# PRBonn/SHINE_mapping

Measured on NVIDIA H100. Metric: sdf_train_points_per_sec_fwd_bwd, higher is better.
Workload: dtype f32

## Files before the change

shine_mapping_b200/csrc/shine_b200.cu:

```cuda

#include <cuda_runtime.h>
#include <math.h>
#include <stdint.h>

#include "shine_b200.h"

#ifndef SHINE_GATHER_GROUP
#define SHINE_GATHER_GROUP 2
#endif
#ifndef SHINE_TRAIN_MINB
#define SHINE_TRAIN_MINB 2
#endif
#ifndef SHINE_TRAIN_DECGRAD_MINB
#define SHINE_TRAIN_DECGRAD_MINB 1
#endif
#ifndef SHINE_INFER_MINB
#define SHINE_INFER_MINB 3
#endif

#include "shine_device.cuh"

namespace {


// ... 222 lines not shown
    const float s0 = odd ? v[0] : v[2], s1 = odd ? v[1] : v[3];
    const float r0 = __shfl_xor_sync(kFull, s0, 1), r1 = __shfl_xor_sync(kFull, s1, 1);
    if (!odd) { a[0] = v[0]; a[2] = v[1]; a[1] = r0; a[3] = r1; }
    else      { a[0] = r0;   a[2] = r1;   a[1] = v[2]; a[3] = v[3]; }
}
__device__ __forceinline__ void from_cfrag(const float (&c)[4], int odd, float (&v)[4]) {
    const float s0 = odd ? c[0] : c[2], s1 = odd ? c[1] : c[3];
    const float r0 = __shfl_xor_sync(kFull, s0, 1), r1 = __shfl_xor_sync(kFull, s1, 1);
    if (!odd) { v[0] = c[0]; v[1] = c[1]; v[2] = r0; v[3] = r1; }
    else      { v[0] = r0;   v[1] = r1;   v[2] = c[2]; v[3] = c[3]; }
}

#define SHINE_ACC_DECL float dW2[2][4][4], dW1[2][4], db2p[4][2], db1p[4][2], dw3p[4][2]

__device__ __forceinline__ float reduce_scatter_g8(const float (&v)[8], int lane) {
    float a[4], b[2];
    const bool b4 = (lane & 16) != 0, b3 = (lane & 8) != 0, b2 = (lane & 4) != 0;
#pragma unroll
    for (int i = 0; i < 4; ++i) a[i] = (b4 ? v[4 + i] : v[i]) + __shfl_xor_sync(kFull, b4 ? v[i] : v[4 + i], 16);
#pragma unroll
    for (int i = 0; i < 2; ++i) b[i] = (b3 ? a[2 + i] : a[i]) + __shfl_xor_sync(kFull, b3 ? a[i] : a[2 + i], 8);
    return (b2 ? b[1] : b[0]) + __shfl_xor_sync(kFull, b2 ? b[0] : b[1], 4);
}

__device__ __forceinline__ int frag_chunk(int lane) { return lane ^ ((lane >> 2) & 6); }
template <int NTF>
__device__ __forceinline__ void load_afrag(const float* blk, int c, AFrag<NTF>& a) {
    const float4 v = *reinterpret_cast<const float4*>(blk + 4 * c);
    a.set_packed(v.x, v.y, v.z, v.w);
}
__device__ __forceinline__ void load_bfrag(const float* blk, int c, uint2& bh, uint2& bl) {
    const float2 v = *reinterpret_cast<const float2*>(blk + 2 * c);
    split_fast2(v.x, v.y, bh.x, bh.y, bl.x, bl.y);
}
__device__ __forceinline__ void stage_afrags(float* blk, const int (&sq)[2], const float (&c)[4][4]) {
#pragma unroll
    for (int mt = 0; mt < 2; ++mt)
#pragma unroll
        for (int q = 0; q < 2; ++q)
            *reinterpret_cast<float4*>(blk + 128 * mt + 4 * sq[q]) = make_float4(c[2 * mt][q], c[2 * mt + 1][q], c[2 * mt][2 + q], c[2 * mt + 1][2 + q]);
}
__device__ __forceinline__ int xfrag_word(int ks, int c) { return 64 * ks + 2 * (c ^ (8 * ks)); }
__device__ __forceinline__ void load_xfrag(const float* sx, int ks, int c, uint2& bh, uint2& bl) {
    const float2 v = *reinterpret_cast<const float2*>(sx + xfrag_word(ks, c));
    split_fast2(v.x, v.y, bh.x, bh.y, bl.x, bl.y);
}


constexpr int kGatherGroup = SHINE_GATHER_GROUP;

using shine_internal::StepParams;

struct SmemPlan {
    static constexpr int W1 = 0;
    static constexpr int W1T = W1 + 2 * kH * kF;
    static constexpr int W2 = W1T + 2 * kF * kWS;
    static constexpr int W3W2T = W2 + 2 * kH * kWS;
    static constexpr int B1 = W3W2T + 2 * kH * kWS;
    static constexpr int B2 = B1 + kH;
    static constexpr int W3 = B2 + kH;
    static constexpr int B3 = W3 + kH;
    static constexpr int GSCALE = B3 + 1;
    static constexpr int kDecGradFloats = kH * kF + kH + kH * kH + kH + kH + 1;
    static constexpr int ZSUM = B3 + 4;
    static constexpr int kZsumFloats = 8 * 5 * kTile;
    static constexpr int STAGE = ZSUM + kZsumFloats;
    static constexpr int SB2 = 0;
    static constexpr int SU = SB2;
    static constexpr int SA1 = SB2 + kTile * kH;
    static constexpr int SX = SA1 + kTile * kH;
    static constexpr int SA2 = SX + kTile * kF;
    static constexpr int SDP = SA2;
    static constexpr int kStagePerWarp = SA2 + kTile * kH;
    static constexpr int kStageGrouped = SDP + 2 * kTile;
    __host__ __device__ static constexpr int stage_per_warp(bool grouped) { return grouped ? kStageGrouped : kStagePerWarp; }
    static constexpr int kGroupPerLevel = 4 * kTile;
    static constexpr int kW2Part = kH * kH;
};

constexpr int kMaxGroupedRuns = 6;

__device__ __forceinline__ void red_add_f2(float* p, float a, float b) {
    asm volatile("red.global.add.v2.f32 [%0], {%1,%2};" ::"l"(p), "f"(a), "f"(b) : "memory");
}
__device__ __forceinline__ int group_slot(int p) { return 4 * (p & 3) + (p >> 2); }

template <int LMAX>
__device__ __forceinline__ void grouped_scatter(const StepParams& P, int L, int tile, const float* __restrict__ pt,
                                                float* __restrict__ dtile, const float (&dxc)[4], int lane) {
    const int g = lane >> 2, t = lane & 3;
    *reinterpret_cast<float2*>(dtile + g * kF + 2 * t) = make_float2(dxc[0], dxc[1]);
    *reinterpret_cast<float2*>(dtile + (g + 8) * kF + 2 * t) = make_float2(dxc[2], dxc[3]);
    __syncwarp();
    uint2 bh[2], bl[2];
#pragma unroll
    for (int c = 0; c < 2; ++c)
        split_fast2(dtile[(8 * c + t) * kF + g], dtile[(8 * c + t + 4) * kF + g], bh[c].x, bh[c].y, bl[c].x, bl[c].y);
    const float sx = (g & 4) ? 1.f : -1.f, ox = (g & 4) ? 0.f : 1.f;
    const float sy = (g & 2) ? 1.f : -1.f, oy = (g & 2) ? 0.f : 1.f;
    const float sz = (g & 1) ? 1.f : -1.f, oz = (g & 1) ? 0.f : 1.f;
    const int id_off = 8 * (g & 1) + 4 + (g >> 1);
    const int own = group_slot(lane & 15);
#pragma unroll
    for (int i = 0; i < LMAX; ++i) {
        if (i >= L) break;
        const float* lt = pt + i * SmemPlan::kGroupPerLevel;
        const int v_own = __float_as_int(lt[48 + own]);
        const uint32_t same = __match_any_sync(kFull, v_own);
        const int lead = __ffs(same) - 1;
        const uint32_t bmask = __ballot_sync(kFull, v_own >= 0 && lead == lane);
        if (bmask == 0) continue;
        const int rid_own = v_own >= 0 ? __popc(bmask & ((1u << lead) - 1u)) : 255;
        const shine_level& lv = P.oct.lv[i];
        const int32_t* slot_words = reinterpret_cast<const int32_t*>(lv.hash_slots);
        float* gb = grad_base(lv, (uint32_t)tile, kF);
        const int nruns = __popc(bmask);
        if (nruns > kMaxGroupedRuns) {
            const int odd = t & 1, half = t >> 1, mp = group_slot(g + 8 * odd);
// ... 28 lines not shown
        {
            const f2_t s_x = f2_pack(sx, sx), o_x = f2_pack(ox, ox), s_y = f2_pack(sy, sy), o_y = f2_pack(oy, oy);
            const f2_t s_z = f2_pack(sz, sz), o_z = f2_pack(oz, oz);
            const f2_t X01 = f2_fma(f2_pack(tx4.x, tx4.y), s_x, o_x), X23 = f2_fma(f2_pack(tx4.z, tx4.w), s_x, o_x);
            const f2_t Y01 = f2_fma(f2_pack(ty4.x, ty4.y), s_y, o_y), Y23 = f2_fma(f2_pack(ty4.z, ty4.w), s_y, o_y);
            const f2_t Z01 = f2_fma(f2_pack(tz4.x, tz4.y), s_z, o_z), Z23 = f2_fma(f2_pack(tz4.z, tz4.w), s_z, o_z);
            f2_unpack(f2_mul(f2_mul(X01, Y01), Z01), w[0], w[1]);
            f2_unpack(f2_mul(f2_mul(X23, Y23), Z23), w[2], w[3]);
        }
        int rid[4];
#pragma unroll
        for (int q = 0; q < 4; ++q) rid[q] = __shfl_sync(kFull, rid_own, t + 4 * q);
        uint32_t rem = bmask;
        for (int r = 0; r < nruns; r += 2) {
            const int p1 = __ffs(rem) - 1; rem &= rem - 1;
            const int p2 = rem ? __ffs(rem) - 1 : p1; rem &= rem - 1;
            const int v1 = __shfl_sync(kFull, v_own, p1);
            const int v2 = (r + 1 < nruns) ? __shfl_sync(kFull, v_own, p2) : -1;
            AFrag<3> a0, a1;
            a0.set(rid[0] == r ? w[0] : 0.f, rid[0] == r + 1 ? w[0] : 0.f, rid[1] == r ? w[1] : 0.f, rid[1] == r + 1 ? w[1] : 0.f);
            a1.set(rid[2] == r ? w[2] : 0.f, rid[2] == r + 1 ? w[2] : 0.f, rid[3] == r ? w[3] : 0.f, rid[3] == r + 1 ? w[3] : 0.f);
            float c0[4] = {0.f, 0.f, 0.f, 0.f}, c1[4] = {0.f, 0.f, 0.f, 0.f};
            mma3x2<3>(c0, c1, a0, a1, bh[0], bl[0], bh[1], bl[1]);
            if (v1 >= 0) {
                const int row = __ldg(slot_words + 16 * (int64_t)v1 + id_off);
                red_add_f2(gb + (int64_t)row * kF + 2 * t, c0[0] + c1[0], c0[1] + c1[1]);
            }
            if (v2 >= 0) {
                const int row = __ldg(slot_words + 16 * (int64_t)v2 + id_off);
                red_add_f2(gb + (int64_t)row * kF + 2 * t, c0[2] + c1[2], c0[3] + c1[3]);
            }
        }
    }
    __syncwarp();
}

template <int NTF, bool TRAIN, bool DEC_GRAD, int LMAX, bool GROUPED = false>
__global__ void __launch_bounds__(256, !TRAIN ? SHINE_INFER_MINB : (DEC_GRAD && !GROUPED) ? SHINE_TRAIN_DECGRAD_MINB : SHINE_TRAIN_MINB)
sdf_fused_kernel(const __grid_constant__ StepParams P) {
    static_assert(!GROUPED || TRAIN, "the grouped scatter belongs to the training kernels");
    static_assert(!DEC_GRAD || TRAIN, "decoder gradients belong to the training kernels");
    static_assert(SmemPlan::kStagePerWarp >= SmemPlan::kDecGradFloats, "a warp's staging area holds its partial decoder gradient");
    static_assert(SmemPlan::kStageGrouped >= kH * kF + 3 * kH + 1, "a grouped warp's staging area holds its partial bias / dW1 gradients");
    static_assert(!(GROUPED && DEC_GRAD) ||
                      (SmemPlan::STAGE + 8 * (SmemPlan::kStageGrouped + LMAX * SmemPlan::kGroupPerLevel + SmemPlan::kW2Part)) * 4 + 1024 <=
                          227 * 1024 / SHINE_TRAIN_MINB,
                  "the grouped kernel's shared memory fits SHINE_TRAIN_MINB blocks/SM");
    extern __shared__ __align__(16) float smem[];
    uint32_t* smu = reinterpret_cast<uint32_t*>(smem);
    const int tid = threadIdx.x, lane = tid & 31, warp = tid >> 5;
    const int g = lane >> 2, t = lane & 3, odd = t & 1, half = t >> 1;
    constexpr int kWarps = 8;

    for (int i = tid; i < kH * kF; i += blockDim.x) {
        const int nrow = i / kF, k = i % kF;
        uint32_t hi, lo; split_tf32(P.dec.w1[i], hi, lo);
        smu[SmemPlan::W1 + i] = hi; smu[SmemPlan::W1 + kH * kF + i] = lo;
        smu[SmemPlan::W1T + k * kWS + nrow] = hi; smu[SmemPlan::W1T + kF * kWS + k * kWS + nrow] = lo;
    }
    for (int i = tid; i < kH * kH; i += blockDim.x) {
        const int nrow = i / kH, k = i % kH;
        const float w = P.dec.w2[i];
        uint32_t hi, lo; split_tf32(w, hi, lo);
        smu[SmemPlan::W2 + nrow * kWS + k] = hi; smu[SmemPlan::W2 + kH * kWS + nrow * kWS + k] = lo;
        split_tf32(__fmul_rn(P.dec.w3[nrow], w), hi, lo);
        smu[SmemPlan::W3W2T + k * kWS + nrow] = hi; smu[SmemPlan::W3W2T + kH * kWS + k * kWS + nrow] = lo;
    }
    if (tid < kH) {
        smem[SmemPlan::B1 + tid] = P.dec.b1 ? P.dec.b1[tid] : 0.f;
        smem[SmemPlan::B2 + tid] = P.dec.b2 ? P.dec.b2[tid] : 0.f;
        smem[SmemPlan::W3 + tid] = P.dec.w3[tid];
    }
    if (tid == 0) {
        smem[SmemPlan::B3] = P.dec.b3 ? P.dec.b3[0] : 0.f;
        smem[SmemPlan::GSCALE] = P.loss_scale * ((TRAIN && P.d_loss) ? __ldg(P.d_loss) : 1.0f);
    }
    constexpr int kPark = LMAX <= 4 ? 16 : 32;
    constexpr int kIdPark = 4 * LMAX;
    __syncthreads();
    SHINE_ACC_DECL;
#pragma unroll
    for (int a = 0; a < 2; ++a) {
#pragma unroll
        for (int b = 0; b < 4; ++b) { dW2[a][b][0] = dW2[a][b][1] = dW2[a][b][2] = dW2[a][b][3] = 0.f; }
        dW1[a][0] = dW1[a][1] = dW1[a][2] = dW1[a][3] = 0.f;
    }
#pragma unroll
    for (int j = 0; j < 4; ++j) { db2p[j][0] = db2p[j][1] = db1p[j][0] = db1p[j][1] = dw3p[j][0] = dw3p[j][1] = 0.f; }
    float dw3acc = 0.f, db2acc[4] = {0.f, 0.f, 0.f, 0.f}, db1acc[2][2] = {{0.f, 0.f}, {0.f, 0.f}};

    constexpr bool kSectorProbe = !TRAIN;
    const bool poly = P.oct.poly_interp != 0;
    const int L = P.oct.num_levels;

    float db3p = 0.f;
    float loss_acc = 0.f;

    constexpr int kStage = SmemPlan::stage_per_warp(GROUPED);
    float* stage = smem + SmemPlan::STAGE + warp * kStage;
    float* stX = stage + SmemPlan::SX;
    const int kp = g >> 2, fc = frag_chunk(lane);
    const int sq[2] = {frag_chunk(8 * t + (g & 3)), frag_chunk(8 * t + 4 + (g & 3))};
    float* gpt = smem + SmemPlan::STAGE + (DEC_GRAD ? 8 * kStage : 0) +
                 warp * (LMAX * SmemPlan::kGroupPerLevel + (DEC_GRAD ? 0 : kTile * kF));
    float* gdx = DEC_GRAD ? stX : gpt + LMAX * SmemPlan::kGroupPerLevel;
    float* w2p = smem + SmemPlan::STAGE + 8 * kStage + 8 * LMAX * SmemPlan::kGroupPerLevel + warp * SmemPlan::kW2Part;
    if (DEC_GRAD && GROUPED) {
#pragma unroll
        for (int f = 0; f < 8; ++f) *reinterpret_cast<float4*>(w2p + 128 * f + 4 * lane) = make_float4(0.f, 0.f, 0.f, 0.f);
    }

    const int warp_global = blockIdx.x * kWarps + warp;
    const int warp_stride = gridDim.x * kWarps;

    bool consecutive = true;
#pragma unroll
    for (int i = 1; i < LMAX; ++i)
        if (i < L && P.oct.lv[i].level != P.oct.lv[0].level - i) consecutive = false;

// ... 165 lines not shown
            for (int i = 0; i < kIdPark; ++i) idp[i] = __int_as_float(-1);
#pragma unroll
            for (int i = 0; i < LMAX; ++i) {
                if (GROUPED && i < L && half) gpt[i * SmemPlan::kGroupPerLevel + 48 + group_slot(g + 8 * odd)] = __int_as_float(slot[i]);
                if (i < L && slot[i] >= 0) {
                    const shine_level& lv = P.oct.lv[i];
                    const HashSlot* slots = reinterpret_cast<const HashSlot*>(lv.hash_slots);
                    hitmask |= 1u << i;
                    const int4 id4 = ldg_i4(slot_ids(slots, slot[i], half));
                    idp[4 * i] = __int_as_float(id4.x); idp[4 * i + 1] = __int_as_float(id4.y);
                    idp[4 * i + 2] = __int_as_float(id4.z); idp[4 * i + 3] = __int_as_float(id4.w);
                    float r0[8], r1[8], r2[8], r3[8];
                    ldg_row8(lv.features + (int64_t)id4.x * kF, r0);
                    ldg_row8(lv.features + (int64_t)id4.y * kF, r1);
                    ldg_row8(lv.features + (int64_t)id4.z * kF, r2);
                    ldg_row8(lv.features + (int64_t)id4.w * kF, r3);
                    Blend b; b.init(x, y, z, lv.level, poly);
                    pk[3 * i] = b.tx; pk[3 * i + 1] = b.ty; pk[3 * i + 2] = b.tz;
                    if (GROUPED) {
                        float* lt = gpt + i * SmemPlan::kGroupPerLevel + group_slot(g + 8 * odd);
                        if (half) lt[32] = b.tz; else { lt[0] = b.tx; lt[16] = b.ty; }
                    }
                    const float wz = half ? b.tz : b.uz;
                    const float w0 = __fmul_rn(__fmul_rn(b.ux, b.uy), wz), w1 = __fmul_rn(__fmul_rn(b.ux, b.ty), wz);
                    const float w2 = __fmul_rn(__fmul_rn(b.tx, b.uy), wz), w3 = __fmul_rn(__fmul_rn(b.tx, b.ty), wz);
                    blend4(acc, r0, r1, r2, r3, w0, w1, w2, w3);
                }
            }
#pragma unroll
            for (int q = 0; q < 4; ++q) {
                const float send = half ? acc[q] : acc[4 + q];
                const float recv = __shfl_xor_sync(kFull, send, 2);
                feat[q] = (half ? acc[4 + q] : acc[q]) + recv;
            }
        }
        }
        if (phase == 1 && __ballot_sync(kFull, hitmask != 0u) == 0u) {
            if (!TRAIN && P.mask && half == 0 && valid) P.mask[myp] = 0;
            if (P.pred && half == 0 && valid) P.pred[myp] = pred0;
            if (P.label != nullptr && valid) {
                float li, dpz;
                bce_point(pred0, lab, wgt, li, dpz);
                if (half == 0) { loss_acc += wgt * li; zsum += dpz; }
            }
            continue;
        }
        if (!TRAIN && P.mask) {
            bool present = false;
#pragma unroll
            for (int i = 0; i < LMAX; ++i) present = (i == P.mask_level) ? (((hitmask >> i) & 1u) != 0) : present;
            if (half == 0 && valid) P.mask[myp] = (uint8_t)present;
        }

        AFrag<NTF> ax;
        {
            float a[4]; to_afrag(feat, odd, a);
            ax.set(a[0], a[1], a[2], a[3]);
        }
        if (DEC_GRAD) {
#pragma unroll
            for (int q = 0; q < 4; ++q) stX[xfrag_word(kp, frag_chunk(16 * half + 4 * q + (g & 3))) + odd] = feat[q];
        }
        float h1[4][4];
        uint32_t m1 = 0;
        {
            uint2 bh[4], bl[4];
#pragma unroll
            for (int j = 0; j < 4; ++j) {
                const float bA = smem[SmemPlan::B1 + 8 * j + 2 * t], bB = smem[SmemPlan::B1 + 8 * j + 2 * t + 1];
                h1[j][0] = bA; h1[j][1] = bB; h1[j][2] = bA; h1[j][3] = bB;
                const int off = (8 * j + g) * kF + 2 * t;
                bh[j] = *reinterpret_cast<const uint2*>(smu + SmemPlan::W1 + off);
                bl[j] = *reinterpret_cast<const uint2*>(smu + SmemPlan::W1 + kH * kF + off);
            }
            mma3x4<NTF>(h1, ax, bh, bl);
#pragma unroll
            for (int j = 0; j < 4; ++j) {
#pragma unroll
                for (int r = 0; r < 4; ++r) {
                    if (TRAIN && h1[j][r] > 0.f) m1 |= 1u << (4 * j + r);
                    h1[j][r] = fmaxf(h1[j][r], 0.f);
                }
                if (DEC_GRAD && !GROUPED) {
#pragma unroll
                    for (int q = 0; q < 2; ++q)
                        *reinterpret_cast<float2*>(stage + SmemPlan::SB2 + (4 * kp + j) * 64 + 2 * sq[q]) = make_float2(h1[j][q], h1[j][2 + q]);
                }
            }
            if (DEC_GRAD && GROUPED) stage_afrags(stage + SmemPlan::SU + 256 * kp, sq, h1);
        }
        float h2[4][4];
        {
#pragma unroll
            for (int j = 0; j < 4; ++j) {
                const float bA = smem[SmemPlan::B2 + 8 * j + 2 * t], bB = smem[SmemPlan::B2 + 8 * j + 2 * t + 1];
                h2[j][0] = bA; h2[j][1] = bB; h2[j][2] = bA; h2[j][3] = bB;
            }
#pragma unroll
            for (int kk = 0; kk < 4; ++kk) {
                AFrag<NTF> a; a.set(h1[kk][0], h1[kk][2], h1[kk][1], h1[kk][3]);
                uint2 bh[4], bl[4];
#pragma unroll
                for (int j = 0; j < 4; ++j) {
                    const int off = (8 * j + g) * kWS + 8 * kk + 2 * t;
                    bh[j] = *reinterpret_cast<const uint2*>(smu + SmemPlan::W2 + off);
                    bl[j] = *reinterpret_cast<const uint2*>(smu + SmemPlan::W2 + kH * kWS + off);
                }
                mma3x4<NTF>(h2, a, bh, bl);
            }
#pragma unroll
            for (int j = 0; j < 4; ++j) {
#pragma unroll
                for (int r = 0; r < 4; ++r) h2[j][r] = fmaxf(h2[j][r], 0.f);
            }
        }
        float w3a[4], w3b[4];
#pragma unroll
        for (int j = 0; j < 4; ++j) { w3a[j] = smem[SmemPlan::W3 + 8 * j + 2 * t]; w3b[j] = smem[SmemPlan::W3 + 8 * j + 2 * t + 1]; }
        float p0 = 0.f, p8 = 0.f;
#pragma unroll
        for (int j = 0; j < 4; ++j) {
            p0 = fmaf(h2[j][0], w3a[j], p0); p0 = fmaf(h2[j][1], w3b[j], p0);
            p8 = fmaf(h2[j][2], w3a[j], p8); p8 = fmaf(h2[j][3], w3b[j], p8);
        }
        p0 += __shfl_xor_sync(kFull, p0, 1); p0 += __shfl_xor_sync(kFull, p0, 2);
        p8 += __shfl_xor_sync(kFull, p8, 1); p8 += __shfl_xor_sync(kFull, p8, 2);
        const float b3 = smem[SmemPlan::B3];
        p0 += b3; p8 += b3;
        const float pown = odd ? p8 : p0;
        if (phase == 0) { pred0 = pown; phase = 1; continue; }
        if (P.pred && half == 0 && valid) P.pred[myp] = pown;

        if (P.label == nullptr) continue;

        float dpo = 0.f;
        if (valid) {
            float li;
            bce_point(pown, lab, wgt, li, dpo);
            if (half == 0) loss_acc += wgt * li;
        }
        if (!TRAIN) continue;
        if (phase == 2) dpo = (g == 0 && odd == 0) ? zsum : 0.f;

        const float dpx = __shfl_xor_sync(kFull, dpo, 1);
        const float dp0 = odd ? dpx : dpo, dp8 = odd ? dpo : dpx;
        float db1t[4][2], dw3t[4][2];
        if (DEC_GRAD) {
#pragma unroll
            for (int j = 0; j < 4; ++j) { dw3t[j][0] = dp0 * h2[j][0] + dp8 * h2[j][2];  dw3t[j][1] = dp0 * h2[j][1] + dp8 * h2[j][3]; }
        }
        if (DEC_GRAD && !GROUPED) {
            float dh2[4][4];
#pragma unroll
            for (int j = 0; j < 4; ++j) {
                dh2[j][0] = h2[j][0] > 0.f ? dp0 * w3a[j] : 0.f; dh2[j][1] = h2[j][1] > 0.f ? dp0 * w3b[j] : 0.f;
                dh2[j][2] = h2[j][2] > 0.f ? dp8 * w3a[j] : 0.f; dh2[j][3] = h2[j][3] > 0.f ? dp8 * w3b[j] : 0.f;
                db2p[j][0] += dh2[j][0] + dh2[j][2]; db2p[j][1] += dh2[j][1] + dh2[j][3];
            }
            stage_afrags(stage + SmemPlan::SA2 + 256 * kp, sq, dh2);
        }
        if (DEC_GRAD && GROUPED) {
            uint32_t mg = 0, mg8 = 0;
#pragma unroll
            for (int j = 0; j < 4; ++j)
#pragma unroll
                for (int q = 0; q < 2; ++q) {
                    mg |= (h2[j][q] > 0.f ? 1u : 0u) << (8 * j + 2 * t + q);
                    mg8 |= (h2[j][2 + q] > 0.f ? 1u : 0u) << (8 * j + 2 * t + q);
                }
            mg |= __shfl_xor_sync(kFull, mg, 1); mg8 |= __shfl_xor_sync(kFull, mg8, 1);
            mg |= __shfl_xor_sync(kFull, mg, 2); mg8 |= __shfl_xor_sync(kFull, mg8, 2);
            if (t == 0) {
                *reinterpret_cast<float2*>(stage + SmemPlan::SDP + 2 * g) = make_float2(dp0, __uint_as_float(mg));
                *reinterpret_cast<float2*>(stage + SmemPlan::SDP + 2 * (g + 8)) = make_float2(dp8, __uint_as_float(mg8));
            }
        }
        if (DEC_GRAD && t == 0) db3p += dp0 + dp8;

        float dh1[4][4];
        {
#pragma unroll
            for (int j = 0; j < 4; ++j) { dh1[j][0] = dh1[j][1] = dh1[j][2] = dh1[j][3] = 0.f; }
#pragma unroll
            for (int kk = 0; kk < 4; ++kk) {
                const uint32_t a[4] = {h2[kk][0] > 0.f ? kTf32One : 0u, h2[kk][2] > 0.f ? kTf32One : 0u,
                                       h2[kk][1] > 0.f ? kTf32One : 0u, h2[kk][3] > 0.f ? kTf32One : 0u};
                uint2 bh[4], bl[4];
#pragma unroll
                for (int j = 0; j < 4; ++j) {
                    const int off = (8 * j + g) * kWS + 8 * kk + 2 * t;
                    bh[j] = *reinterpret_cast<const uint2*>(smu + SmemPlan::W3W2T + off);
                    bl[j] = *reinterpret_cast<const uint2*>(smu + SmemPlan::W3W2T + kH * kWS + off);
                }
                mma2x4_exact_a<NTF>(dh1, a, bh, bl);
            }
#pragma unroll
            for (int j = 0; j < 4; ++j) {
                dh1[j][0] *= dp0; dh1[j][1] *= dp0; dh1[j][2] *= dp8; dh1[j][3] *= dp8;
#pragma unroll
                for (int r = 0; r < 4; ++r) dh1[j][r] = ((m1 >> (4 * j + r)) & 1u) ? dh1[j][r] : 0.f;
                if (DEC_GRAD) { db1t[j][0] = dh1[j][0] + dh1[j][2]; db1t[j][1] = dh1[j][1] + dh1[j][3]; }
            }
            if (DEC_GRAD) stage_afrags(stage + SmemPlan::SA1 + 256 * kp, sq, dh1);
        }
        float dxc[4] = {0.f, 0.f, 0.f, 0.f};
        {
            float dxo[4] = {0.f, 0.f, 0.f, 0.f};
#pragma unroll
            for (int kk = 0; kk < 4; kk += 2) {
                AFrag<NTF> a0, a1;
                a0.set(dh1[kk][0], dh1[kk][2], dh1[kk][1], dh1[kk][3]);
                a1.set(dh1[kk + 1][0], dh1[kk + 1][2], dh1[kk + 1][1], dh1[kk + 1][3]);
                const int off = g * kWS + 8 * kk + 2 * t;
                const uint2 bh0 = *reinterpret_cast<const uint2*>(smu + SmemPlan::W1T + off);
                const uint2 bl0 = *reinterpret_cast<const uint2*>(smu + SmemPlan::W1T + kF * kWS + off);
                const uint2 bh1 = *reinterpret_cast<const uint2*>(smu + SmemPlan::W1T + off + 8);
                const uint2 bl1 = *reinterpret_cast<const uint2*>(smu + SmemPlan::W1T + kF * kWS + off + 8);
                mma3x2<NTF>(dxc, dxo, a0, a1, bh0, bl0, bh1, bl1);
            }
#pragma unroll
            for (int r = 0; r < 4; ++r) dxc[r] += dxo[r];
        }

        if (DEC_GRAD && !GROUPED) {
#pragma unroll
            for (int j = 0; j < 4; ++j) {
                db1p[j][0] += db1t[j][0]; db1p[j][1] += db1t[j][1];
                dw3p[j][0] += dw3t[j][0]; dw3p[j][1] += dw3t[j][1];
            }
            __syncwarp();
#pragma unroll
            for (int ks = 0; ks < 2; ++ks) {
                uint2 bh[4], bl[4];
#pragma unroll
                for (int nt = 0; nt < 4; ++nt) load_bfrag(stage + SmemPlan::SB2 + (4 * ks + nt) * 64, fc, bh[nt], bl[nt]);
#pragma unroll
                for (int mt = 0; mt < 2; ++mt) {
                    AFrag<NTF> a;
                    load_afrag(stage + SmemPlan::SA2 + (2 * ks + mt) * 128, fc, a);
                    mma3x4<NTF>(dW2[mt], a, bh, bl);
                }
            }
#pragma unroll
            for (int ks = 0; ks < 2; ++ks) {
                uint2 bh, bl;
                load_xfrag(stX, ks, fc, bh, bl);
                AFrag<NTF> a0, a1;
                load_afrag(stage + SmemPlan::SA1 + (2 * ks) * 128, fc, a0);
                load_afrag(stage + SmemPlan::SA1 + (2 * ks + 1) * 128, fc, a1);
                mma3x2<NTF>(dW1[0], dW1[1], a0, a1, bh, bl, bh, bl);
            }
            __syncwarp();
        }
        if (DEC_GRAD && GROUPED) {
            float cols[8];
#pragma unroll
            for (int j = 0; j < 4; ++j) { cols[2 * j] = dw3t[j][0]; cols[2 * j + 1] = dw3t[j][1]; }
            dw3acc += reduce_scatter_g8(cols, lane);
            __syncwarp();
// ... 627 lines not shown
```

shine_mapping_b200/csrc/shine_device.cuh:

```cuda
#pragma once

#include <cuda_runtime.h>
#include <math.h>
#include <stdint.h>

#include "shine_b200.h"

namespace shine_internal {

struct StepParams {
    shine_octree oct;
    shine_decoder dec;
    const float* coord;
    const float* label;
    const float* weight;
    const float* d_loss;
    float* pred;
    float* loss;
    uint8_t* mask;
    int64_t n;
    int32_t num_tiles;
    int32_t mask_level;
    float sigma;
    float loss_scale;
// ... 253 lines not shown
__device__ __forceinline__ void blend4(float (&acc)[8], const float (&r0)[8], const float (&r1)[8], const float (&r2)[8],
                                       const float (&r3)[8], float w0, float w1, float w2, float w3) {
    const f2_t p0 = f2_pack(w0, w0), p1 = f2_pack(w1, w1), p2 = f2_pack(w2, w2), p3 = f2_pack(w3, w3);
#pragma unroll
    for (int q = 0; q < 8; q += 2) {
        f2_t a = f2_pack(acc[q], acc[q + 1]);
        a = f2_fma(p0, f2_pack(r0[q], r0[q + 1]), a); a = f2_fma(p1, f2_pack(r1[q], r1[q + 1]), a);
        a = f2_fma(p2, f2_pack(r2[q], r2[q + 1]), a); a = f2_fma(p3, f2_pack(r3[q], r3[q + 1]), a);
        f2_unpack(a, acc[q], acc[q + 1]);
    }
}

template <int NTF>
__device__ __forceinline__ void mma3x4(float (&d)[4][4], const AFrag<NTF>& a, const uint2 (&bh)[4], const uint2 (&bl)[4]) {
    if (NTF == 3) {
#pragma unroll
        for (int j = 0; j < 4; ++j) mma_tf32(d[j], a.lo, bh[j].x, bh[j].y);
#pragma unroll
        for (int j = 0; j < 4; ++j) mma_tf32(d[j], a.hi, bl[j].x, bl[j].y);
    }
#pragma unroll
    for (int j = 0; j < 4; ++j) mma_tf32(d[j], a.hi, bh[j].x, bh[j].y);
}
template <int NTF>
__device__ __forceinline__ void mma3x2(float (&d0)[4], float (&d1)[4], const AFrag<NTF>& a0, const AFrag<NTF>& a1,
                                       uint2 bh0, uint2 bl0, uint2 bh1, uint2 bl1) {
    if (NTF == 3) {
        mma_tf32(d0, a0.lo, bh0.x, bh0.y); mma_tf32(d1, a1.lo, bh1.x, bh1.y);
        mma_tf32(d0, a0.hi, bl0.x, bl0.y); mma_tf32(d1, a1.hi, bl1.x, bl1.y);
    }
    mma_tf32(d0, a0.hi, bh0.x, bh0.y); mma_tf32(d1, a1.hi, bh1.x, bh1.y);
}
constexpr uint32_t kTf32One = 0x3f800000u;
template <int NTF>
__device__ __forceinline__ void mma2x4_exact_a(float (&d)[4][4], const uint32_t (&a)[4], const uint2 (&bh)[4], const uint2 (&bl)[4]) {
    if (NTF == 3) {
#pragma unroll
        for (int j = 0; j < 4; ++j) mma_tf32(d[j], a, bl[j].x, bl[j].y);
    }
#pragma unroll
    for (int j = 0; j < 4; ++j) mma_tf32(d[j], a, bh[j].x, bh[j].y);
}
template <int NTF>
__device__ __forceinline__ void mma2x4_exact_b(float (&d)[4][4], const AFrag<NTF>& a, const uint2 (&b)[4]) {
    if (NTF == 3) {
#pragma unroll
        for (int j = 0; j < 4; ++j) mma_tf32(d[j], a.lo, b[j].x, b[j].y);
    }
#pragma unroll
    for (int j = 0; j < 4; ++j) mma_tf32(d[j], a.hi, b[j].x, b[j].y);
}


constexpr int kMaxDevices = 64;

inline bool is_pow2(uint32_t v) { return v && !(v & (v - 1)); }

struct DeviceGuard {
    int prev = -1, dev = -1;
    bool switched = false;
    explicit DeviceGuard(const void* p) {
        if (cudaGetDevice(&prev) != cudaSuccess) { prev = -1; (void)cudaGetLastError(); }
        dev = prev;
        if (!p) return;
        cudaPointerAttributes a;
        if (cudaPointerGetAttributes(&a, p) != cudaSuccess) { (void)cudaGetLastError(); return; }
        if (a.type != cudaMemoryTypeDevice && a.type != cudaMemoryTypeManaged) return;
        dev = a.device;
        if (dev != prev && cudaSetDevice(dev) == cudaSuccess) switched = true;
    }
    ~DeviceGuard() { if (switched) (void)cudaSetDevice(prev); }
    DeviceGuard(const DeviceGuard&) = delete;
    DeviceGuard& operator=(const DeviceGuard&) = delete;
};

inline int device_of(const void* p) {
    if (!p) return -1;
    cudaPointerAttributes a;
    if (cudaPointerGetAttributes(&a, p) != cudaSuccess) { (void)cudaGetLastError(); return -1; }
    return (a.type == cudaMemoryTypeDevice || a.type == cudaMemoryTypeManaged) ? a.device : -1;
}

inline int current_device() {
    int dev = 0;
    if (cudaGetDevice(&dev) != cudaSuccess || dev < 0 || dev >= kMaxDevices) return 0;
    return dev;
}

inline int sm_count() {
    static int cached[kMaxDevices] = {0};
    const int dev = current_device();
    if (cached[dev] == 0) {
        int n = 0;
        if (cudaDeviceGetAttribute(&n, cudaDevAttrMultiProcessorCount, dev) != cudaSuccess || n <= 0) n = 132;
        cached[dev] = n;
    }
    return cached[dev];
}

inline int check_octree(const shine_octree* o, bool need_grads) {
    if (!o) return SHINE_ERR_INVALID_ARG;
    if (o->num_levels < 1 || o->num_levels > SHINE_MAX_LEVELS) return SHINE_ERR_INVALID_ARG;
    if (o->feature_dim < 4 || (o->feature_dim & 3)) return SHINE_ERR_UNSUPPORTED;
    for (int i = 0; i < o->num_levels; ++i) {
        const shine_level& lv = o->lv[i];
        if (!lv.hash_slots || !lv.features || !is_pow2(lv.hash_capacity) || lv.rows < 1) return SHINE_ERR_INVALID_ARG;
// ... 15 lines not shown
```

Measured before the change: 4.157 billion.

## Replace 3xTF32 decoder MMAs with scaled split-FP16 m16n8k16 MMAs

```diff
diff --git a/shine_mapping_b200/csrc/shine_b200.cu b/shine_mapping_b200/csrc/shine_b200.cu
--- a/shine_mapping_b200/csrc/shine_b200.cu
+++ b/shine_mapping_b200/csrc/shine_b200.cu
@@ -298,6 +298,10 @@
 using shine_internal::StepParams;
 
 struct SmemPlan {
+    static constexpr int F16W1 = 0;
+    static constexpr int F16W2 = F16W1 + 4 * 32 * 2;
+    static constexpr int F16W3W2 = F16W2 + 2 * 4 * 32 * 4;
+    static constexpr int F16W1T = F16W3W2 + 2 * 4 * 32 * 4;
     static constexpr int W1 = 0;
     static constexpr int W1T = W1 + 2 * kH * kF;
     static constexpr int W2 = W1T + 2 * kF * kWS;
@@ -310,6 +314,8 @@
     static constexpr int kDecGradFloats = kH * kF + kH + kH * kH + kH + kH + 1;
     static constexpr int ZSUM = B3 + 4;
     static constexpr int kZsumFloats = 8 * 5 * kTile;
+    static constexpr int F16UNS = ZSUM + 8;
+    static constexpr int F16MAX = F16UNS + 4;
     static constexpr int STAGE = ZSUM + kZsumFloats;
     static constexpr int SB2 = 0;
     static constexpr int SU = SB2;
@@ -444,19 +450,70 @@
     const int g = lane >> 2, t = lane & 3, odd = t & 1, half = t >> 1;
     constexpr int kWarps = 8;
 
-    for (int i = tid; i < kH * kF; i += blockDim.x) {
-        const int nrow = i / kF, k = i % kF;
-        uint32_t hi, lo; split_tf32(P.dec.w1[i], hi, lo);
-        smu[SmemPlan::W1 + i] = hi; smu[SmemPlan::W1 + kH * kF + i] = lo;
-        smu[SmemPlan::W1T + k * kWS + nrow] = hi; smu[SmemPlan::W1T + kF * kWS + k * kWS + nrow] = lo;
-    }
-    for (int i = tid; i < kH * kH; i += blockDim.x) {
-        const int nrow = i / kH, k = i % kH;
-        const float w = P.dec.w2[i];
-        uint32_t hi, lo; split_tf32(w, hi, lo);
-        smu[SmemPlan::W2 + nrow * kWS + k] = hi; smu[SmemPlan::W2 + kH * kWS + nrow * kWS + k] = lo;
-        split_tf32(__fmul_rn(P.dec.w3[nrow], w), hi, lo);
-        smu[SmemPlan::W3W2T + k * kWS + nrow] = hi; smu[SmemPlan::W3W2T + kH * kWS + k * kWS + nrow] = lo;
+    if constexpr (NTF == 3) {
+        static_assert(SmemPlan::F16W1T + 2 * 32 * 4 <= SmemPlan::B1, "the f16 fragments fit the weight region");
+        if (tid < 3) smu[SmemPlan::F16MAX + tid] = 0u;
+        __syncthreads();
+        uint32_t m1 = 0, m2 = 0, m32 = 0;
+        for (int i = tid; i < kH * kF; i += blockDim.x) m1 = max(m1, __float_as_uint(P.dec.w1[i]) & 0x7FFFFFFFu);
+        for (int i = tid; i < kH * kH; i += blockDim.x) {
+            const float w = P.dec.w2[i];
+            m2 = max(m2, __float_as_uint(w) & 0x7FFFFFFFu);
+            m32 = max(m32, __float_as_uint(__fmul_rn(P.dec.w3[i / kH], w)) & 0x7FFFFFFFu);
+        }
+        m1 = __reduce_max_sync(kFull, m1); m2 = __reduce_max_sync(kFull, m2); m32 = __reduce_max_sync(kFull, m32);
+        if (lane == 0) {
+            atomicMax(smu + SmemPlan::F16MAX, m1); atomicMax(smu + SmemPlan::F16MAX + 1, m2); atomicMax(smu + SmemPlan::F16MAX + 2, m32);
+        }
+        __syncthreads();
+        const int k1 = f16_scale_exp(smu[SmemPlan::F16MAX] >> 23);
+        const int k2 = f16_scale_exp(smu[SmemPlan::F16MAX + 1] >> 23);
+        const int k32 = f16_scale_exp(smu[SmemPlan::F16MAX + 2] >> 23);
+        const float s1 = exp2i(k1), s2 = exp2i(k2), s32 = exp2i(k32);
+        if (tid < 3) smu[SmemPlan::F16UNS + tid] = (uint32_t)(127 - (tid == 0 ? k1 : tid == 1 ? k2 : k32));
+        for (int i = tid; i < 4 * 32; i += blockDim.x) {
+            const int j = i >> 5, l = i & 31, n = 8 * j + (l >> 2), k = 2 * (l & 3);
+            uint32_t hi, lo; split_f16x2(P.dec.w1[n * kF + k], P.dec.w1[n * kF + k + 1], s1, hi, lo);
+            *reinterpret_cast<uint2*>(smu + SmemPlan::F16W1 + 128 * (j >> 1) + 4 * l + 2 * (j & 1)) = make_uint2(hi, lo);
+        }
+        for (int i = tid; i < 2 * 4 * 32; i += blockDim.x) {
+            const int kk = i >> 7, j = (i >> 5) & 3, l = i & 31, n = 8 * j + (l >> 2), k0 = 16 * kk + 2 * (l & 3);
+            uint4 v;
+            split_f16x2(P.dec.w2[n * kH + k0], P.dec.w2[n * kH + k0 + 1], s2, v.x, v.z);
+            split_f16x2(P.dec.w2[n * kH + k0 + 8], P.dec.w2[n * kH + k0 + 9], s2, v.y, v.w);
+            *reinterpret_cast<uint4*>(smu + SmemPlan::F16W2 + 4 * i) = v;
+            float w[4];
+#pragma unroll
+            for (int q = 0; q < 4; ++q) {
+                const int k = k0 + (q & 1) + 8 * (q >> 1);
+                w[q] = __fmul_rn(P.dec.w3[k], P.dec.w2[k * kH + n]);
+            }
+            split_f16x2(w[0], w[1], s32, v.x, v.z);
+            split_f16x2(w[2], w[3], s32, v.y, v.w);
+            *reinterpret_cast<uint4*>(smu + SmemPlan::F16W3W2 + 4 * i) = v;
+        }
+        for (int i = tid; i < 2 * 32; i += blockDim.x) {
+            const int kk = i >> 5, l = i & 31, n = l >> 2, k0 = 16 * kk + 2 * (l & 3);
+            uint4 v;
+            split_f16x2(P.dec.w1[k0 * kF + n], P.dec.w1[(k0 + 1) * kF + n], s1, v.x, v.z);
+            split_f16x2(P.dec.w1[(k0 + 8) * kF + n], P.dec.w1[(k0 + 9) * kF + n], s1, v.y, v.w);
+            *reinterpret_cast<uint4*>(smu + SmemPlan::F16W1T + 4 * i) = v;
+        }
+    } else {
+        for (int i = tid; i < kH * kF; i += blockDim.x) {
+            const int nrow = i / kF, k = i % kF;
+            uint32_t hi, lo; split_tf32(P.dec.w1[i], hi, lo);
+            smu[SmemPlan::W1 + i] = hi; smu[SmemPlan::W1 + kH * kF + i] = lo;
+            smu[SmemPlan::W1T + k * kWS + nrow] = hi; smu[SmemPlan::W1T + kF * kWS + k * kWS + nrow] = lo;
+        }
+        for (int i = tid; i < kH * kH; i += blockDim.x) {
+            const int nrow = i / kH, k = i % kH;
+            const float w = P.dec.w2[i];
+            uint32_t hi, lo; split_tf32(w, hi, lo);
+            smu[SmemPlan::W2 + nrow * kWS + k] = hi; smu[SmemPlan::W2 + kH * kWS + nrow * kWS + k] = lo;
+            split_tf32(__fmul_rn(P.dec.w3[nrow], w), hi, lo);
+            smu[SmemPlan::W3W2T + k * kWS + nrow] = hi; smu[SmemPlan::W3W2T + kH * kWS + k * kWS + nrow] = lo;
+        }
     }
     if (tid < kH) {
         smem[SmemPlan::B1 + tid] = P.dec.b1 ? P.dec.b1[tid] : 0.f;
@@ -728,11 +785,6 @@
             if (half == 0 && valid) P.mask[myp] = (uint8_t)present;
         }
 
-        AFrag<NTF> ax;
-        {
-            float a[4]; to_afrag(feat, odd, a);
-            ax.set(a[0], a[1], a[2], a[3]);
-        }
         if (DEC_GRAD) {
 #pragma unroll
             for (int q = 0; q < 4; ++q) stX[xfrag_word(kp, frag_chunk(16 * half + 4 * q + (g & 3))) + odd] = feat[q];
@@ -740,16 +792,54 @@
         float h1[4][4];
         uint32_t m1 = 0;
         {
-            uint2 bh[4], bl[4];
-#pragma unroll
-            for (int j = 0; j < 4; ++j) {
-                const float bA = smem[SmemPlan::B1 + 8 * j + 2 * t], bB = smem[SmemPlan::B1 + 8 * j + 2 * t + 1];
-                h1[j][0] = bA; h1[j][1] = bB; h1[j][2] = bA; h1[j][3] = bB;
-                const int off = (8 * j + g) * kF + 2 * t;
-                bh[j] = *reinterpret_cast<const uint2*>(smu + SmemPlan::W1 + off);
-                bl[j] = *reinterpret_cast<const uint2*>(smu + SmemPlan::W1 + kH * kF + off);
-            }
-            mma3x4<NTF>(h1, ax, bh, bl);
+            if constexpr (NTF == 3) {
+                float fm = fmaxf(fmaxf(fabsf(feat[0]), fabsf(feat[1])), fmaxf(fabsf(feat[2]), fabsf(feat[3])));
+                fm = fmaxf(fm, __shfl_xor_sync(kFull, fm, 2));
+                const int kx = f16_scale_exp(__float_as_uint(fm) >> 23);
+                const float sx = exp2i(kx);
+                uint32_t xh[2], xl[2];
+                split_f16x2(feat[0], feat[1], sx, xh[0], xl[0]);
+                split_f16x2(feat[2], feat[3], sx, xh[1], xl[1]);
+                const uint32_t rh = __shfl_xor_sync(kFull, odd ? xh[0] : xh[1], 1);
+                const uint32_t rl = __shfl_xor_sync(kFull, odd ? xl[0] : xl[1], 1);
+                const int kxo = __shfl_xor_sync(kFull, kx, 1);
+                const uint32_t ah[2] = {odd ? rh : xh[0], odd ? xh[1] : rh}, al[2] = {odd ? rl : xl[0], odd ? xl[1] : rl};
+                uint4 bw[2];
+#pragma unroll
+                for (int p = 0; p < 2; ++p) bw[p] = *reinterpret_cast<const uint4*>(smu + SmemPlan::F16W1 + 128 * p + 4 * lane);
+                const uint32_t bh[4] = {bw[0].x, bw[0].z, bw[1].x, bw[1].z}, bl[4] = {bw[0].y, bw[0].w, bw[1].y, bw[1].w};
+                float c[4][4];
+#pragma unroll
+                for (int j = 0; j < 4; ++j) { c[j][0] = c[j][1] = c[j][2] = c[j][3] = 0.f; }
+#pragma unroll
+                for (int j = 0; j < 4; ++j) mma_f16_k8(c[j], al, bh[j]);
+#pragma unroll
+                for (int j = 0; j < 4; ++j) mma_f16_k8(c[j], ah, bl[j]);
+#pragma unroll
+                for (int j = 0; j < 4; ++j) mma_f16_k8(c[j], ah, bh[j]);
+                const int uw = (int)smu[SmemPlan::F16UNS];
+                const float u0 = f16_unscale(odd ? kxo : kx, uw), u8 = f16_unscale(odd ? kx : kxo, uw);
+#pragma unroll
+                for (int j = 0; j < 4; ++j) {
+                    const float bA = smem[SmemPlan::B1 + 8 * j + 2 * t], bB = smem[SmemPlan::B1 + 8 * j + 2 * t + 1];
+                    h1[j][0] = fmaf(c[j][0], u0, bA); h1[j][1] = fmaf(c[j][1], u0, bB);
+                    h1[j][2] = fmaf(c[j][2], u8, bA); h1[j][3] = fmaf(c[j][3], u8, bB);
+                }
+            } else {
+                AFrag<NTF> ax;
+                float a[4]; to_afrag(feat, odd, a);
+                ax.set(a[0], a[1], a[2], a[3]);
+                uint2 bh[4], bl[4];
+#pragma unroll
+                for (int j = 0; j < 4; ++j) {
+                    const float bA = smem[SmemPlan::B1 + 8 * j + 2 * t], bB = smem[SmemPlan::B1 + 8 * j + 2 * t + 1];
+                    h1[j][0] = bA; h1[j][1] = bB; h1[j][2] = bA; h1[j][3] = bB;
+                    const int off = (8 * j + g) * kF + 2 * t;
+                    bh[j] = *reinterpret_cast<const uint2*>(smu + SmemPlan::W1 + off);
+                    bl[j] = *reinterpret_cast<const uint2*>(smu + SmemPlan::W1 + kH * kF + off);
+                }
+                mma3x4<NTF>(h1, ax, bh, bl);
+            }
 #pragma unroll
             for (int j = 0; j < 4; ++j) {
 #pragma unroll
@@ -766,7 +856,37 @@
             if (DEC_GRAD && GROUPED) stage_afrags(stage + SmemPlan::SU + 256 * kp, sq, h1);
         }
         float h2[4][4];
-        {
+        if constexpr (NTF == 3) {
+            float m0 = 0.f, m8 = 0.f;
+#pragma unroll
+            for (int j = 0; j < 4; ++j) { m0 = fmaxf(m0, fmaxf(h1[j][0], h1[j][1])); m8 = fmaxf(m8, fmaxf(h1[j][2], h1[j][3])); }
+            uint32_t e0, e8; quad_row_exps(m0, m8, e0, e8);
+            const int k0 = f16_scale_exp(e0), k8 = f16_scale_exp(e8);
+            const float s0 = exp2i(k0), s8 = exp2i(k8);
+            float c[4][4];
+#pragma unroll
+            for (int j = 0; j < 4; ++j) { c[j][0] = c[j][1] = c[j][2] = c[j][3] = 0.f; }
+#pragma unroll
+            for (int kk = 0; kk < 2; ++kk) {
+                uint32_t ah[4], al[4];
+                split_f16x2(h1[2 * kk][0], h1[2 * kk][1], s0, ah[0], al[0]);
+                split_f16x2(h1[2 * kk][2], h1[2 * kk][3], s8, ah[1], al[1]);
+                split_f16x2(h1[2 * kk + 1][0], h1[2 * kk + 1][1], s0, ah[2], al[2]);
+                split_f16x2(h1[2 * kk + 1][2], h1[2 * kk + 1][3], s8, ah[3], al[3]);
+                uint4 b[4];
+#pragma unroll
+                for (int j = 0; j < 4; ++j) b[j] = *reinterpret_cast<const uint4*>(smu + SmemPlan::F16W2 + 128 * (4 * kk + j) + 4 * lane);
+                mma_f16x4_k16(c, ah, al, b);
+            }
+            const int uw = (int)smu[SmemPlan::F16UNS + 1];
+            const float u0 = f16_unscale(k0, uw), u8 = f16_unscale(k8, uw);
+#pragma unroll
+            for (int j = 0; j < 4; ++j) {
+                const float bA = smem[SmemPlan::B2 + 8 * j + 2 * t], bB = smem[SmemPlan::B2 + 8 * j + 2 * t + 1];
+                h2[j][0] = fmaxf(fmaf(c[j][0], u0, bA), 0.f); h2[j][1] = fmaxf(fmaf(c[j][1], u0, bB), 0.f);
+                h2[j][2] = fmaxf(fmaf(c[j][2], u8, bA), 0.f); h2[j][3] = fmaxf(fmaf(c[j][3], u8, bB), 0.f);
+            }
+        } else {
 #pragma unroll
             for (int j = 0; j < 4; ++j) {
                 const float bA = smem[SmemPlan::B2 + 8 * j + 2 * t], bB = smem[SmemPlan::B2 + 8 * j + 2 * t + 1];
@@ -857,22 +977,38 @@
         {
 #pragma unroll
             for (int j = 0; j < 4; ++j) { dh1[j][0] = dh1[j][1] = dh1[j][2] = dh1[j][3] = 0.f; }
-#pragma unroll
-            for (int kk = 0; kk < 4; ++kk) {
-                const uint32_t a[4] = {h2[kk][0] > 0.f ? kTf32One : 0u, h2[kk][2] > 0.f ? kTf32One : 0u,
-                                       h2[kk][1] > 0.f ? kTf32One : 0u, h2[kk][3] > 0.f ? kTf32One : 0u};
-                uint2 bh[4], bl[4];
-#pragma unroll
-                for (int j = 0; j < 4; ++j) {
-                    const int off = (8 * j + g) * kWS + 8 * kk + 2 * t;
-                    bh[j] = *reinterpret_cast<const uint2*>(smu + SmemPlan::W3W2T + off);
-                    bl[j] = *reinterpret_cast<const uint2*>(smu + SmemPlan::W3W2T + kH * kWS + off);
-                }
-                mma2x4_exact_a<NTF>(dh1, a, bh, bl);
+            float dps0 = dp0, dps8 = dp8;
+            if constexpr (NTF == 3) {
+#pragma unroll
+                for (int kk = 0; kk < 2; ++kk) {
+                    const uint32_t a[4] = {f16_mask2(h2[2 * kk][0] > 0.f, h2[2 * kk][1] > 0.f), f16_mask2(h2[2 * kk][2] > 0.f, h2[2 * kk][3] > 0.f),
+                                           f16_mask2(h2[2 * kk + 1][0] > 0.f, h2[2 * kk + 1][1] > 0.f),
+                                           f16_mask2(h2[2 * kk + 1][2] > 0.f, h2[2 * kk + 1][3] > 0.f)};
+                    uint4 b[4];
+#pragma unroll
+                    for (int j = 0; j < 4; ++j) b[j] = *reinterpret_cast<const uint4*>(smu + SmemPlan::F16W3W2 + 128 * (4 * kk + j) + 4 * lane);
+                    mma_f16x4_k16_exact_a(dh1, a, b);
+                }
+                const float u = f16_unscale(0, (int)smu[SmemPlan::F16UNS + 2]);
+                dps0 = dp0 * u; dps8 = dp8 * u;
+            } else {
+#pragma unroll
+                for (int kk = 0; kk < 4; ++kk) {
+                    const uint32_t a[4] = {h2[kk][0] > 0.f ? kTf32One : 0u, h2[kk][2] > 0.f ? kTf32One : 0u,
+                                           h2[kk][1] > 0.f ? kTf32One : 0u, h2[kk][3] > 0.f ? kTf32One : 0u};
+                    uint2 bh[4], bl[4];
+#pragma unroll
+                    for (int j = 0; j < 4; ++j) {
+                        const int off = (8 * j + g) * kWS + 8 * kk + 2 * t;
+                        bh[j] = *reinterpret_cast<const uint2*>(smu + SmemPlan::W3W2T + off);
+                        bl[j] = *reinterpret_cast<const uint2*>(smu + SmemPlan::W3W2T + kH * kWS + off);
+                    }
+                    mma2x4_exact_a<NTF>(dh1, a, bh, bl);
+                }
             }
 #pragma unroll
             for (int j = 0; j < 4; ++j) {
-                dh1[j][0] *= dp0; dh1[j][1] *= dp0; dh1[j][2] *= dp8; dh1[j][3] *= dp8;
+                dh1[j][0] *= dps0; dh1[j][1] *= dps0; dh1[j][2] *= dps8; dh1[j][3] *= dps8;
 #pragma unroll
                 for (int r = 0; r < 4; ++r) dh1[j][r] = ((m1 >> (4 * j + r)) & 1u) ? dh1[j][r] : 0.f;
                 if (DEC_GRAD) { db1t[j][0] = dh1[j][0] + dh1[j][2]; db1t[j][1] = dh1[j][1] + dh1[j][3]; }
@@ -880,7 +1016,34 @@
             if (DEC_GRAD) stage_afrags(stage + SmemPlan::SA1 + 256 * kp, sq, dh1);
         }
         float dxc[4] = {0.f, 0.f, 0.f, 0.f};
-        {
+        if constexpr (NTF == 3) {
+            float m0 = 0.f, m8 = 0.f;
+#pragma unroll
+            for (int j = 0; j < 4; ++j) {
+                m0 = fmaxf(m0, fmaxf(fabsf(dh1[j][0]), fabsf(dh1[j][1]))); m8 = fmaxf(m8, fmaxf(fabsf(dh1[j][2]), fabsf(dh1[j][3])));
+            }
+            uint32_t e0, e8; quad_row_exps(m0, m8, e0, e8);
+            const int k0 = f16_scale_exp(e0), k8 = f16_scale_exp(e8);
+            const float s0 = exp2i(k0), s8 = exp2i(k8);
+            uint32_t ah[2][4], al[2][4];
+            uint4 b[2];
+#pragma unroll
+            for (int kk = 0; kk < 2; ++kk) {
+                split_f16x2(dh1[2 * kk][0], dh1[2 * kk][1], s0, ah[kk][0], al[kk][0]);
+                split_f16x2(dh1[2 * kk][2], dh1[2 * kk][3], s8, ah[kk][1], al[kk][1]);
+                split_f16x2(dh1[2 * kk + 1][0], dh1[2 * kk + 1][1], s0, ah[kk][2], al[kk][2]);
+                split_f16x2(dh1[2 * kk + 1][2], dh1[2 * kk + 1][3], s8, ah[kk][3], al[kk][3]);
+                b[kk] = *reinterpret_cast<const uint4*>(smu + SmemPlan::F16W1T + 128 * kk + 4 * lane);
+            }
+            float dxo[4] = {0.f, 0.f, 0.f, 0.f};
+            mma_f16_k16(dxc, al[0], b[0].x, b[0].y); mma_f16_k16(dxo, al[1], b[1].x, b[1].y);
+            mma_f16_k16(dxc, ah[0], b[0].z, b[0].w); mma_f16_k16(dxo, ah[1], b[1].z, b[1].w);
+            mma_f16_k16(dxc, ah[0], b[0].x, b[0].y); mma_f16_k16(dxo, ah[1], b[1].x, b[1].y);
+            const int uw = (int)smu[SmemPlan::F16UNS];
+            const float u0 = f16_unscale(k0, uw), u8 = f16_unscale(k8, uw);
+            dxc[0] = (dxc[0] + dxo[0]) * u0; dxc[1] = (dxc[1] + dxo[1]) * u0;
+            dxc[2] = (dxc[2] + dxo[2]) * u8; dxc[3] = (dxc[3] + dxo[3]) * u8;
+        } else {
             float dxo[4] = {0.f, 0.f, 0.f, 0.f};
 #pragma unroll
             for (int kk = 0; kk < 4; kk += 2) {
diff --git a/shine_mapping_b200/csrc/shine_device.cuh b/shine_mapping_b200/csrc/shine_device.cuh
--- a/shine_mapping_b200/csrc/shine_device.cuh
+++ b/shine_mapping_b200/csrc/shine_device.cuh
@@ -329,6 +329,65 @@
 }
 
 
+__device__ __forceinline__ uint32_t f16x2_rn(float x0, float x1) {
+    uint32_t r;
+    asm("cvt.rn.f16x2.f32 %0, %1, %2;" : "=r"(r) : "f"(x1), "f"(x0));
+    return r;
+}
+__device__ __forceinline__ float2 f16x2_to_f32(uint32_t v) {
+    float a, b;
+    asm("{.reg .f16 l, h;\n\tmov.b32 {l, h}, %2;\n\tcvt.f32.f16 %0, l;\n\tcvt.f32.f16 %1, h;}" : "=f"(a), "=f"(b) : "r"(v));
+    return make_float2(a, b);
+}
+__device__ __forceinline__ float exp2i(int k) { return __uint_as_float((uint32_t)(k + 127) << 23); }
+__device__ __forceinline__ void split_f16x2(float x0, float x1, float s, uint32_t& hi, uint32_t& lo) {
+    const float y0 = x0 * s, y1 = x1 * s;
+    hi = f16x2_rn(y0, y1);
+    const float2 h = f16x2_to_f32(hi);
+    lo = f16x2_rn(y0 - h.x, y1 - h.y);
+}
+constexpr int kF16MaxExp = 62;
+__device__ __forceinline__ int f16_scale_exp(uint32_t e) {
+    return min(max(e ? 141 - (int)e : 0, -kF16MaxExp), kF16MaxExp);
+}
+__device__ __forceinline__ float f16_unscale(int kA, int unscale_bias) { return __uint_as_float((uint32_t)(unscale_bias - kA) << 23); }
+__device__ __forceinline__ void quad_row_exps(float m0, float m8, uint32_t& e0, uint32_t& e8) {
+    uint32_t p = __byte_perm(__float_as_uint(m0), __float_as_uint(m8), 0x7632);
+    p = __vmaxu2(p, __shfl_xor_sync(kFull, p, 1));
+    p = __vmaxu2(p, __shfl_xor_sync(kFull, p, 2));
+    e0 = (p >> 7) & 0xFFu; e8 = p >> 23;
+}
+constexpr uint32_t kF16One = 0x3C00u;
+__device__ __forceinline__ uint32_t f16_mask2(bool m0, bool m1) { return (m0 ? kF16One : 0u) | (m1 ? kF16One << 16 : 0u); }
+
+__device__ __forceinline__ void mma_f16_k16(float (&d)[4], const uint32_t (&a)[4], uint32_t b0, uint32_t b1) {
+    asm volatile(
+        "mma.sync.aligned.m16n8k16.row.col.f32.f16.f16.f32 {%0,%1,%2,%3}, {%4,%5,%6,%7}, {%8,%9}, {%0,%1,%2,%3};"
+        : "+f"(d[0]), "+f"(d[1]), "+f"(d[2]), "+f"(d[3])
+        : "r"(a[0]), "r"(a[1]), "r"(a[2]), "r"(a[3]), "r"(b0), "r"(b1));
+}
+__device__ __forceinline__ void mma_f16_k8(float (&d)[4], const uint32_t (&a)[2], uint32_t b) {
+    asm volatile(
+        "mma.sync.aligned.m16n8k8.row.col.f32.f16.f16.f32 {%0,%1,%2,%3}, {%4,%5}, {%6}, {%0,%1,%2,%3};"
+        : "+f"(d[0]), "+f"(d[1]), "+f"(d[2]), "+f"(d[3])
+        : "r"(a[0]), "r"(a[1]), "r"(b));
+}
+__device__ __forceinline__ void mma_f16x4_k16(float (&d)[4][4], const uint32_t (&ah)[4], const uint32_t (&al)[4], const uint4 (&b)[4]) {
+#pragma unroll
+    for (int j = 0; j < 4; ++j) mma_f16_k16(d[j], al, b[j].x, b[j].y);
+#pragma unroll
+    for (int j = 0; j < 4; ++j) mma_f16_k16(d[j], ah, b[j].z, b[j].w);
+#pragma unroll
+    for (int j = 0; j < 4; ++j) mma_f16_k16(d[j], ah, b[j].x, b[j].y);
+}
+__device__ __forceinline__ void mma_f16x4_k16_exact_a(float (&d)[4][4], const uint32_t (&a)[4], const uint4 (&b)[4]) {
+#pragma unroll
+    for (int j = 0; j < 4; ++j) mma_f16_k16(d[j], a, b[j].z, b[j].w);
+#pragma unroll
+    for (int j = 0; j < 4; ++j) mma_f16_k16(d[j], a, b[j].x, b[j].y);
+}
+
+
 constexpr int kMaxDevices = 64;
 
 inline bool is_pow2(uint32_t v) { return v && !(v & (v - 1)); }
```

Result: faster. 4.218 billion, median of 6 (+1.5%).
